# tomoyoshki/focal

Hardware: AMD Instinct MI355X
Metric: pretrain windows/sec (whole node), FOCAL SW_Transformer (higher is better)
Workload: dtype bf16

## Files before the change

### focal_amd/csrc/fft.hip

```cpp
#include <stdlib.h>
#include <type_traits>
#include "common.hpp"

struct AugParams {
  float scale, pc, ps;
  int flip, use_perm;
  int perm[FOCAL_AUG_MAX_INTERVALS];
  const focal_view_plan* plan;
  const float* x_alt;
};
static AugParams aug_identity() {
  AugParams a;
  memset(&a, 0, sizeof(a));
  a.scale = 1.f; a.pc = 1.f;
  return a;
}
struct AugLive {
  float scale, pc, ps;
  int flip, use_perm;
  const float* x;
};
__device__ __forceinline__ AugLive aug_resolve(const AugParams& a, const float* x, int* s_perm, int tid) {
  AugLive v{a.scale, a.pc, a.ps, a.flip, a.use_perm, x};
  if (a.plan != nullptr) {
    const focal_view_plan* pl = a.plan;
    v.scale = pl->aug.scale; v.pc = pl->aug.phase_cos; v.ps = pl->aug.phase_sin;
    v.flip = pl->aug.flip != 0; v.use_perm = pl->aug.use_perm != 0;
    if (focal_plan_warp(pl) != 0) v.x = a.x_alt;
    if (tid < FOCAL_AUG_MAX_INTERVALS) s_perm[tid] = pl->aug.perm[tid];
  } else if (tid < FOCAL_AUG_MAX_INTERVALS) {
    s_perm[tid] = a.perm[tid];
  }
  return v;
}
__device__ __forceinline__ int aug_src_row(const AugLive& a, const int* s_perm, int row, int I) {
  const int i = row % I, bc = row / I;
  int j = a.use_perm ? s_perm[i] : i;
  if (a.flip) j = I - 1 - j;
  return bc * I + j;
}


struct ExParams { const focal_view_extra* dev; int has; uint32_t salt; focal_view_extra host; };
template <bool EX> struct AugArg : AugParams {};
template <> struct AugArg<true> : AugParams { ExParams ex; };
struct ExLive {
  float std; uint32_t key;
  int any, use_chan, tlo, thi, flo, fhi;
};
__device__ __forceinline__ ExLive ex_resolve(const ExParams& p, int C, int n, int* s_chan, int tid) {
  float sd = 0.f;
  uint32_t key = 0u;
  int uc = 0, tlo = 0, tn = 0, flo = 0, fn = 0, ch = tid;
  if (p.dev != nullptr) {
    const focal_view_extra* e = p.dev;
    sd = e->jitter_std; key = e->jitter_key; uc = e->use_chan; tlo = e->tmask_lo; tn = e->tmask_n; flo = e->fmask_lo; fn = e->fmask_n;
    if (tid < FOCAL_VIEW_MAX_CHANNELS) ch = e->chan[tid];
  } else if (p.has) {
    sd = p.host.jitter_std; key = p.host.jitter_key; uc = p.host.use_chan; tlo = p.host.tmask_lo; tn = p.host.tmask_n;
    flo = p.host.fmask_lo; fn = p.host.fmask_n;
    if (tid < FOCAL_VIEW_MAX_CHANNELS) ch = p.host.chan[tid];
  }
  if (tid < FOCAL_VIEW_MAX_CHANNELS) s_chan[tid] = min(max(ch, 0), C - 1);
  ExLive v;
  v.std = sd > 0.f ? sd : 0.f;
  v.key = focal_mix32(key ^ focal_mix32(p.salt * 0x9E3779B9U + 0x85EBCA6BU));
  v.use_chan = uc != 0 && C <= FOCAL_VIEW_MAX_CHANNELS;
  v.tlo = min(max(tlo, 0), n); v.thi = v.tlo + min(max(tn, 0), n - v.tlo);
  v.flo = min(max(flo, 0), n); v.fhi = v.flo + min(max(fn, 0), n - v.flo);
  v.any = v.std > 0.f || v.use_chan || v.thi > v.tlo || v.fhi > v.flo;
  return v;
}
__device__ __forceinline__ int ex_src_row(const AugLive& a, const ExLive& ex, const int* s_perm, const int* s_chan, int row, int I, int C) {
  const int i = row % I;
  int bc = row / I;
  int j = a.use_perm ? s_perm[i] : i;
  if (a.flip) j = I - 1 - j;
  if (ex.use_chan) {
    const int c = bc % C;
    bc += s_chan[c] - c;
  }
  return bc * I + j;
}
__device__ __forceinline__ void ex_noise_pair(uint32_t k, uint32_t p, float& z0, float& z1) {
  const float u1 = 1.0f - (focal_mix32(k + (2u * p) * 0x85EBCA6BU) >> 8) * (1.0f / 16777216.0f);
  const float u2 = (focal_mix32(k + (2u * p + 1u) * 0x85EBCA6BU) >> 8) * (1.0f / 16777216.0f);
  const float r = sqrtf(-2.0f * __logf(u1)), a = 6.283185307179586f * u2;
  z0 = r * __cosf(a);
  z1 = r * __sinf(a);
}
__device__ __forceinline__ float ex_noise(uint32_t k, uint32_t e) {
  float z0, z1;
  ex_noise_pair(k, e >> 1, z0, z1);
  return (e & 1u) ? z1 : z0;
}

typedef float f4 __attribute__((ext_vector_type(4)));
__device__ __forceinline__ f4 mfma4(float a, float b, f4 c) { return __builtin_amdgcn_mfma_f32_16x16x4f32(a, b, c, 0, 0, 0); }

#define FFT_MULTI_MAX 8
struct FftSmallProblem { const float* x; const float* tw; float* out; int rows, I, n, rpb; AugParams aug; };
struct FftSmallExtraProblem : FftSmallProblem { int C; ExParams ex; };
template <bool EX> struct FftSmallTable { int nprob; int wg_end[FFT_MULTI_MAX]; std::conditional_t<EX, FftSmallExtraProblem, FftSmallProblem> p[FFT_MULTI_MAX]; };
static_assert(sizeof(FftSmallTable<true>) <= 4096, "the problem table travels in the kernel arguments");

template <bool EX>
__global__ __launch_bounds__(256) void fft_realpack_kernel(const float* __restrict__ x_arg, const float* __restrict__ tw,
                                                           float* __restrict__ out, focal_fft_desc d, int rows, AugArg<EX> aug_arg) {
  extern __shared__ __attribute__((aligned(16))) float smem[];
  __shared__ int s_perm[FOCAL_AUG_MAX_INTERVALS];
  const AugLive aug = aug_resolve(aug_arg, x_arg, s_perm, threadIdx.x);
  const float* x = aug.x;
  const int n = d.n, n1 = d.n1, n2 = d.n2;
  const int* s_chan = nullptr;
  ExLive ex{};
  if constexpr (EX) {
    __shared__ int chan_tab[FOCAL_VIEW_MAX_CHANNELS];
    ex = ex_resolve(aug_arg.ex, d.C, n, chan_tab, threadIdx.x);
    s_chan = chan_tab;
  }
  float* xs = smem;
  float* yr = smem + n;
  float* yi = yr + n;
  float* twc = yi + n;
  float* tws = twc + n;
  const int tid = threadIdx.x;
  for (int i = tid; i < n; i += 256) {
    twc[i] = tw[2 * i];
    tws[i] = tw[2 * i + 1];
  }
  for (int row = blockIdx.x; row < rows; row += gridDim.x) {
    __syncthreads();
    if (EX && ex.any) {
      const float* xr = x + (long)ex_src_row(aug, ex, s_perm, s_chan, row, d.I, d.C) * n;
      const uint32_t e0 = (uint32_t)row * (uint32_t)n;
      for (int i = tid; i < n; i += 256) {
        float v = aug.scale * xr[aug.flip ? n - 1 - i : i];
        if (ex.std > 0.f) v += ex.std * ex_noise(ex.key, e0 + (uint32_t)i);
        xs[i] = (i >= ex.tlo && i < ex.thi) ? 0.f : v;
      }
    } else {
      const float* xr = x + (long)aug_src_row(aug, s_perm, row, d.I) * n;
      for (int i = tid; i < n; i += 256) xs[i] = aug.scale * xr[aug.flip ? n - 1 - i : i];
    }
    __syncthreads();
    for (int o = tid; o < n; o += 256) {
      const int m2 = o / n1, k1 = o % n1;
      float re = 0.f, im = 0.f;
      int ph = 0;
      for (int m1 = 0; m1 < n1; ++m1) {
        const float v = xs[n2 * m1 + m2];
        re += v * twc[ph * n2];
        im += v * tws[ph * n2];
        ph += k1;
        if (ph >= n1) ph -= n1;
      }
      const int t = (m2 * k1) % n;
      const float c = twc[t], s = tws[t];
      yr[o] = re * c - im * s;
      yi[o] = re * s + im * c;
    }
    __syncthreads();
    const int ci = row % d.I, bc = row / d.I;
    float* ore = out + ((long)(2 * bc) * d.I + ci) * n;
    float* oim = out + ((long)(2 * bc + 1) * d.I + ci) * n;
    for (int o = tid; o < n; o += 256) {
      const int k = o, k1 = k % n1, k2 = k / n1;
      float re = 0.f, im = 0.f;
      int ph = 0;
      for (int m2 = 0; m2 < n2; ++m2) {
        const float a = yr[m2 * n1 + k1], b = yi[m2 * n1 + k1];
        const float c = twc[ph * n1], s = tws[ph * n1];
        re += a * c - b * s;
        im += a * s + b * c;
        ph += k2;
        if (ph >= n2) ph -= n2;
      }
      float orr = re * aug.pc - im * aug.ps, oii = re * aug.ps + im * aug.pc;
      if (EX && k >= ex.flo && k < ex.fhi) orr = oii = 0.f;
      ore[k] = orr;
      oim[k] = oii;
    }
  }
}
template <int N1, int N2, bool EX>
__global__ __launch_bounds__(256) void fft_realpack_mfma_kernel(const float* __restrict__ x_arg, const float* __restrict__ tw,
                                                                float* __restrict__ out, focal_fft_desc d, int rows, AugArg<EX> aug_arg) {
  constexpr int P = 48;
  extern __shared__ __attribute__((aligned(16))) float smem[];
  __shared__ int s_perm[FOCAL_AUG_MAX_INTERVALS];
  const AugLive aug = aug_resolve(aug_arg, x_arg, s_perm, threadIdx.x);
  const float* x = aug.x;
  constexpr int n = N1 * N2, n1 = N1, n2 = N2;
  const int* s_chan = nullptr;
  ExLive ex{};
  if constexpr (EX) {
    __shared__ int chan_tab[FOCAL_VIEW_MAX_CHANNELS];
    ex = ex_resolve(aug_arg.ex, d.C, n, chan_tab, threadIdx.x);
    s_chan = chan_tab;
  }
  float* twc = smem;
  float* tws = twc + n;
  float* w1c = tws + n;
  float* w1s = w1c + n1 * P;
  constexpr bool same = n1 == n2;
  float* w2c = same ? w1c : w1s + n1 * P;
  float* w2s = same ? w1s : w2c + n2 * P;
  float* yr = (same ? w1s : w2s) + n2 * P;
  float* yi = yr + 2 * n2 * P;
  float* xs = yi + 2 * n2 * P;
  const int tid = threadIdx.x, lane = tid & 63, wave = tid >> 6;
  const int lj = lane & 15, lg = lane >> 4;
  for (int i = tid; i < n; i += 256) { twc[i] = tw[2 * i]; tws[i] = tw[2 * i + 1]; }
  for (int i = tid; i < n1 * P; i += 256) {
    const int m = i / P, k = i % P;
    const int t = ((m * k) % n1) * n2;
    w1c[i] = k < n1 ? tw[2 * t] : 0.f;
    w1s[i] = k < n1 ? tw[2 * t + 1] : 0.f;
  }
  for (int i = tid; i < (same ? 0 : n2 * P); i += 256) {
    const int m = i / P, k = i % P;
    const int t = ((m * k) % n2) * n1;
    w2c[i] = k < n2 ? tw[2 * t] : 0.f;
    w2s[i] = k < n2 ? tw[2 * t + 1] : 0.f;
  }
  constexpr int mt1 = 2 * n2 / 16, mt2 = 2 * n1 / 16;
  constexpr int XV = (2 * n / 4 + 255) / 256;
  float4 xn[XV];
  auto fetch = [&](int pair) {
#pragma unroll
    for (int i = 0; i < XV; ++i) {
      const int e = tid + 256 * i;
      float4 v = make_float4(0.f, 0.f, 0.f, 0.f);
      if (e < 2 * n / 4 && pair < rows / 2) {
        const int rl = e / (n / 4), q = e - rl * (n / 4);
        const int srow = (EX && ex.any) ? ex_src_row(aug, ex, s_perm, s_chan, pair * 2 + rl, d.I, d.C) : aug_src_row(aug, s_perm, pair * 2 + rl, d.I);
        const float4* src = reinterpret_cast<const float4*>(x + (long)srow * n);
        if (aug.flip) {
          const float4 t = src[n / 4 - 1 - q];
          v = make_float4(t.w, t.z, t.y, t.x);
        } else {
          v = src[q];
        }
        v.x *= aug.scale; v.y *= aug.scale; v.z *= aug.scale; v.w *= aug.scale;
        if (EX && ex.any) {
          if (ex.std > 0.f) {
            const uint32_t p0 = ((uint32_t)(pair * 2 + rl) * (uint32_t)n + 4u * (uint32_t)q) >> 1;
            float z0, z1, z2, z3;
            ex_noise_pair(ex.key, p0, z0, z1);
            ex_noise_pair(ex.key, p0 + 1u, z2, z3);
            v.x += ex.std * z0; v.y += ex.std * z1; v.z += ex.std * z2; v.w += ex.std * z3;
          }
          const int i0 = 4 * q;
          if (i0 >= ex.tlo && i0 < ex.thi) v.x = 0.f;
          if (i0 + 1 >= ex.tlo && i0 + 1 < ex.thi) v.y = 0.f;
          if (i0 + 2 >= ex.tlo && i0 + 2 < ex.thi) v.z = 0.f;
          if (i0 + 3 >= ex.tlo && i0 + 3 < ex.thi) v.w = 0.f;
        }
      }
      xn[i] = v;
    }
  };
  auto stash = [&]() {
#pragma unroll
    for (int i = 0; i < XV; ++i) {
      const int e = tid + 256 * i;
      if (e < 2 * n / 4) reinterpret_cast<float4*>(xs)[e] = xn[i];
    }
  };
  __syncthreads();
  fetch(blockIdx.x);
  stash();
  for (int pair = blockIdx.x; pair < rows / 2; pair += gridDim.x) {
    __syncthreads();
    const float* x0 = xs;
    constexpr int np1 = (n1 + 15) / 16, np2 = (n2 + 15) / 16;
    for (int u = wave; u < mt1 * np1; u += 4) {
      const int mt = u / np1, p = u - mt * np1;
      const int f = 16 * mt + lj, row = f / n2, m2 = f - row * n2;
      const float* xa = x0 + row * n + m2;
      float a[12];
#pragma unroll
      for (int ks = 0; ks < 12; ++ks) {
        const int m1 = 4 * ks + lg;
        a[ks] = m1 < n1 ? xa[n2 * m1] : 0.f;
      }
      {
        f4 re = {0.f, 0.f, 0.f, 0.f}, im = re, re2 = re, im2 = re;
#pragma unroll
        for (int ks = 0; ks < 12; ks += 2) {
          if (4 * ks >= n1) break;
          const int bi = (4 * ks + lg) * P + 16 * p + lj;
          re = mfma4(a[ks], w1c[bi], re);
          im = mfma4(a[ks], w1s[bi], im);
          if (4 * (ks + 1) < n1) {
            re2 = mfma4(a[ks + 1], w1c[bi + 4 * P], re2);
            im2 = mfma4(a[ks + 1], w1s[bi + 4 * P], im2);
          }
        }
        re += re2;
        im += im2;
        const int k1 = 16 * p + lj;
        if (k1 < n1) {
#pragma unroll
          for (int r = 0; r < 4; ++r) {
            const int fo = 16 * mt + 4 * lg + r, ro = fo / n2, mo = fo - ro * n2;
            const int t = (mo * k1) % n;
            const float c = twc[t], sn = tws[t];
            yr[(ro * n2 + mo) * P + k1] = re[r] * c - im[r] * sn;
            yi[(ro * n2 + mo) * P + k1] = re[r] * sn + im[r] * c;
          }
        }
      }
    }
    __syncthreads();
    fetch(pair + gridDim.x);
    for (int u = wave; u < mt2 * np2; u += 4) {
      const int mt = u / np2, p = u - mt * np2;
      const int f = 16 * mt + lj, row = f / n1, k1 = f - row * n1;
      const float* ya = yr + row * n2 * P + k1;
      const float* yb = yi + row * n2 * P + k1;
      const int fo = 16 * mt + 4 * lg, ro = fo / n1, ko = fo - ro * n1;
      const int grow = pair * 2 + ro;
      const int ci = grow % d.I, bc = grow / d.I;
      float* ore = out + ((long)(2 * bc) * d.I + ci) * n + ko;
      float* oim = out + ((long)(2 * bc + 1) * d.I + ci) * n + ko;
      {
        f4 re = {0.f, 0.f, 0.f, 0.f}, im = re, re2 = re, im2 = re;
#pragma unroll
        for (int ks = 0; ks < 12; ++ks) {
          if (4 * ks >= n2) break;
          const int m2 = 4 * ks + lg;
          const float ar = ya[m2 * P], ai = yb[m2 * P];
          const int bi = m2 * P + 16 * p + lj;
          const float c = w2c[bi], sn = w2s[bi];
          re = mfma4(ar, c, re);
          im = mfma4(ar, sn, im);
          re2 = mfma4(ai, -sn, re2);
          im2 = mfma4(ai, c, im2);
        }
        re += re2;
        im += im2;
        const int k2 = 16 * p + lj;
        if (k2 < n2) {
          f4 orr = re * aug.pc - im * aug.ps, oii = re * aug.ps + im * aug.pc;
          if (EX && ex.fhi > ex.flo) {
#pragma unroll
            for (int r = 0; r < 4; ++r) {
              const int k = ko + r + n1 * k2;
              if (k >= ex.flo && k < ex.fhi) { orr[r] = 0.f; oii[r] = 0.f; }
            }
          }
          *reinterpret_cast<float4*>(ore + n1 * k2) = make_float4(orr[0], orr[1], orr[2], orr[3]);
          *reinterpret_cast<float4*>(oim + n1 * k2) = make_float4(oii[0], oii[1], oii[2], oii[3]);
        }
      }
    }
    stash();
  }
}
template <bool EX>
__global__ __launch_bounds__(256) void fft_small_multi_kernel(const FftSmallTable<EX> t) {
  __shared__ float xs[256], twc[64], tws[64];
  const int b = blockIdx.x, tid = threadIdx.x;
  int pi = 0;
#pragma unroll
  for (int q = 0; q < FFT_MULTI_MAX - 1; ++q) pi += (q < t.nprob - 1 && b >= t.wg_end[q]) ? 1 : 0;
  const auto& P = t.p[pi];
  __shared__ int s_perm[FOCAL_AUG_MAX_INTERVALS];
  const AugLive aug = aug_resolve(P.aug, P.x, s_perm, tid);
  int Cc = 1;
  const int* s_chan = nullptr;
  ExLive ex{};
  if constexpr (EX) {
    __shared__ int chan_tab[FOCAL_VIEW_MAX_CHANNELS];
    Cc = P.C;
    ex = ex_resolve(P.ex, Cc, P.n, chan_tab, threadIdx.x);
    s_chan = chan_tab;
  }
  const int start = pi > 0 ? t.wg_end[pi - 1] : 0, nb = t.wg_end[pi] - start;
  const int n = P.n, rpb = P.rpb;
  if (tid < n) { twc[tid] = P.tw[2 * tid]; tws[tid] = P.tw[2 * tid + 1]; }
  const int r = tid / n, k = tid - r * n;
  const bool active = r < rpb;
  for (int row0 = (b - start) * rpb; row0 < P.rows; row0 += nb * rpb) {
    const int row = row0 + r;
    const bool ok = active && row < P.rows;
    __syncthreads();
    if (EX && ex.any) {
      if (ok) {
        float v = aug.scale * aug.x[(long)ex_src_row(aug, ex, s_perm, s_chan, row, P.I, Cc) * n + (aug.flip ? n - 1 - k : k)];
        if (ex.std > 0.f) v += ex.std * ex_noise(ex.key, (uint32_t)row * (uint32_t)n + (uint32_t)k);
        xs[tid] = (k >= ex.tlo && k < ex.thi) ? 0.f : v;
      }
    } else if (ok) {
      xs[tid] = aug.scale * aug.x[(long)aug_src_row(aug, s_perm, row, P.I) * n + (aug.flip ? n - 1 - k : k)];
    }
    __syncthreads();
    if (!ok) continue;
    const float* xr = xs + r * n;
    float re = 0.f, im = 0.f;
    int ph = 0;
    for (int m = 0; m < n; ++m) {
      const float v = xr[m];
      re += v * twc[ph];
      im += v * tws[ph];
      ph += k;
      if (ph >= n) ph -= n;
    }
    const int ci = row % P.I, bc = row / P.I;
    float orr = re * aug.pc - im * aug.ps, oii = re * aug.ps + im * aug.pc;
    if (EX && k >= ex.flo && k < ex.fhi) orr = oii = 0.f;
    P.out[((long)(2 * bc) * P.I + ci) * n + k] = orr;
    P.out[((long)(2 * bc + 1) * P.I + ci) * n + k] = oii;
  }
}

template <bool EX>
static int fft_launch_t(const focal_fft_desc* d, const AugArg<EX>& aug, const float* x, const float* twiddle, float* out, void* stream) {
  FOCAL_CHECK_ARG(d && x && twiddle && out, "fft_realpack: null argument");
  FOCAL_CHECK_ARG(d->n1 >= 1 && d->n2 >= 1 && d->n1 * d->n2 == d->n, "fft_realpack: n1*n2 != n");
  const size_t sm = (size_t)5 * d->n * sizeof(float);
  FOCAL_CHECK_ARG(sm <= 64 * 1024, "fft_realpack: n=%d too long for the LDS-resident DFT", d->n);
  const int rows = d->B * d->C * d->I;
  const bool mfma_shape = (d->n1 == d->n2) && (d->n1 == 8 || d->n1 == 16 || d->n1 == 24 || d->n1 == 32 || d->n1 == 40 || d->n1 == 48);
  if (mfma_shape && rows % 2 == 0) {
    const size_t smm = (size_t)(2 * d->n + 2 * 48 * d->n1 + (d->n1 == d->n2 ? 0 : 2 * 48 * d->n2) + 4 * 48 * d->n2 + 2 * d->n) * sizeof(float);
    static size_t lds_granted = 48 * 1024;
    if (smm > lds_granted) {
      hipError_t e = hipSuccess;
#define FFT_ATTR(N_) if (e == hipSuccess) e = hipFuncSetAttribute(reinterpret_cast<const void*>(fft_realpack_mfma_kernel<N_, N_, EX>), hipFuncAttributeMaxDynamicSharedMemorySize, (int)smm)
      FFT_ATTR(8); FFT_ATTR(16); FFT_ATTR(24); FFT_ATTR(32); FFT_ATTR(40); FFT_ATTR(48);
#undef FFT_ATTR
      if (e != hipSuccess) {
        focal_set_error("fft_realpack: cannot reserve %zu bytes of LDS: %s", smm, hipGetErrorString(e));
        return FOCAL_EHIP;
      }
      lds_granted = smm;
    }
    const int maxb = 1024;
    int blocks = rows / 2 < maxb ? rows / 2 : maxb;
#define FFT_GO(N_) case N_: FOCAL_LAUNCH((fft_realpack_mfma_kernel<N_, N_, EX>), dim3(blocks), dim3(256), smm, (hipStream_t)stream, x, twiddle, out, *d, rows, aug); break
    switch (d->n1) { FFT_GO(8); FFT_GO(16); FFT_GO(24); FFT_GO(32); FFT_GO(40); default: FFT_GO(48); }
#undef FFT_GO
    FOCAL_LAUNCH_CHECK();
    return FOCAL_OK;
  }
  int blocks = rows < 4096 ? rows : 4096;
  FOCAL_LAUNCH(fft_realpack_kernel<EX>, dim3(blocks), dim3(256), sm, (hipStream_t)stream, x, twiddle, out, *d, rows, aug);
  FOCAL_LAUNCH_CHECK();
  return FOCAL_OK;
}

static int aug_params(const focal_fft_desc* d, const focal_aug_desc* a, AugParams* p) {
  *p = aug_identity();
  if (a == nullptr) return FOCAL_OK;
  p->scale = a->scale;
  p->flip = a->flip != 0;
  p->use_perm = a->use_perm != 0;
  p->pc = a->phase_cos;
  p->ps = a->phase_sin;
  if (p->use_perm) {
    FOCAL_CHECK_ARG(d->I <= FOCAL_AUG_MAX_INTERVALS, "augment_fft: %d intervals exceed the permutation table (%d)", d->I, FOCAL_AUG_MAX_INTERVALS);
    for (int i = 0; i < d->I; ++i) {
      FOCAL_CHECK_ARG(a->perm[i] >= 0 && a->perm[i] < d->I, "augment_fft: permutation entry %d out of range", a->perm[i]);
      p->perm[i] = a->perm[i];
    }
  }
  return FOCAL_OK;
}

static int ex_params(const focal_fft_problem& q, int i, ExParams* e) {
  memset(e, 0, sizeof(*e));
  e->salt = q.noise_salt;
  if (q.extra_dev != nullptr) {
    e->dev = q.extra_dev;
    return FOCAL_OK;
  }
  if (!q.has_extra) return FOCAL_OK;
  const focal_view_extra& x = q.extra;
  const int C = q.d.C, n = q.d.n;
  FOCAL_CHECK_ARG(x.jitter_std >= 0.f, "fft_realpack_multi: negative jitter std in problem %d", i);
  FOCAL_CHECK_ARG(x.tmask_lo >= 0 && x.tmask_n >= 0 && x.tmask_lo <= n && x.tmask_n <= n - x.tmask_lo, "fft_realpack_multi: time mask [%d, +%d) of problem %d leaves [0, %d]", x.tmask_lo, x.tmask_n, i, n);
  FOCAL_CHECK_ARG(x.fmask_lo >= 0 && x.fmask_n >= 0 && x.fmask_lo <= n && x.fmask_n <= n - x.fmask_lo, "fft_realpack_multi: freq mask [%d, +%d) of problem %d leaves [0, %d]", x.fmask_lo, x.fmask_n, i, n);
  if (x.use_chan) {
    FOCAL_CHECK_ARG(C <= FOCAL_VIEW_MAX_CHANNELS, "fft_realpack_multi: %d channels exceed the channel table (%d)", C, FOCAL_VIEW_MAX_CHANNELS);
    unsigned seen = 0;
    for (int c = 0; c < C; ++c) {
      FOCAL_CHECK_ARG(x.chan[c] >= 0 && x.chan[c] < C && !(seen >> x.chan[c] & 1u), "fft_realpack_multi: chan of problem %d is not a permutation of range(%d)", i, C);
      seen |= 1u << x.chan[c];
    }
  }
  e->has = 1;
  e->host = x;
  return FOCAL_OK;
}

template <bool EX>
static int fft_multi(int n, const focal_fft_problem* probs, void* stream) {
  FftSmallTable<EX> t;
  memset(&t, 0, sizeof(t));
  auto flush = [&]() -> int {
    if (t.nprob == 0) return FOCAL_OK;
    FOCAL_LAUNCH(fft_small_multi_kernel<EX>, dim3(t.wg_end[t.nprob - 1]), dim3(256), 0, (hipStream_t)stream, t);
    FOCAL_LAUNCH_CHECK();
    memset(&t, 0, sizeof(t));
    return FOCAL_OK;
  };
  for (int i = 0; i < n; ++i) {
    const focal_fft_problem& q = probs[i];
    FOCAL_CHECK_ARG(q.x && q.twiddle && q.out, "fft_realpack_multi: null tensor in problem %d", i);
    FOCAL_CHECK_ARG(q.d.B > 0 && q.d.C > 0 && q.d.I > 0 && q.d.n > 0, "fft_realpack: bad shape");
    AugArg<EX> ap;
    if (int rc = aug_params(&q.d, q.has_aug ? &q.aug : nullptr, &ap)) return rc;
    if constexpr (EX)
      if (int rc = ex_params(q, i, &ap.ex)) return rc;
    if (q.plan != nullptr) {
      FOCAL_CHECK_ARG(q.x_warped != nullptr && q.d.I <= FOCAL_AUG_MAX_INTERVALS, "fft_realpack_multi: a device plan needs x_warped and at most %d intervals", FOCAL_AUG_MAX_INTERVALS);
      ap.plan = q.plan;
      ap.x_alt = q.x_warped;
    }
    if (q.d.n <= 64 && q.d.n2 == 1 && q.d.n1 == q.d.n) {
      auto& P = t.p[t.nprob];
      if constexpr (EX) { P.C = q.d.C; P.ex = ap.ex; }
      P.x = q.x; P.tw = q.twiddle; P.out = q.out;
      P.rows = q.d.B * q.d.C * q.d.I; P.I = q.d.I; P.n = q.d.n; P.rpb = 256 / q.d.n;
      P.aug = ap;
      int blocks = ceil_div(P.rows, P.rpb);
      if (blocks > 1024) blocks = 1024;
      t.wg_end[t.nprob] = (t.nprob ? t.wg_end[t.nprob - 1] : 0) + blocks;
      if (++t.nprob == FFT_MULTI_MAX)
        if (int rc = flush()) return rc;
    } else if (int rc = fft_launch_t<EX>(&q.d, ap, q.x, q.twiddle, q.out, stream)) {
      return rc;
    }
  }
  return flush();
}

extern "C" int focal_fft_realpack_multi(int n, const focal_fft_problem* probs, void* stream) {
  FOCAL_CHECK_ARG(n >= 1 && probs, "fft_realpack_multi: no problems");
  bool ex = false;
  for (int i = 0; i < n; ++i) ex = ex || probs[i].has_extra || probs[i].extra_dev != nullptr;
  return ex ? fft_multi<true>(n, probs, stream) : fft_multi<false>(n, probs, stream);
}

extern "C" int focal_fft_realpack_fwd(const focal_fft_desc* d, const float* x, const float* twiddle, float* out, void* stream) {
  return fft_launch_t<false>(d, AugArg<false>{aug_identity()}, x, twiddle, out, stream);
}

extern "C" int focal_augment_fft_fwd(const focal_fft_desc* d, const focal_aug_desc* a, const float* x, const float* twiddle, float* out,
                                     void* stream) {
  FOCAL_CHECK_ARG(d && a, "augment_fft: null descriptor");
  AugArg<false> p;
  if (int rc = aug_params(d, a, &p)) return rc;
  return fft_launch_t<false>(d, p, x, twiddle, out, stream);
}
```

Measured before the change: 51920.

## Keep DFT twiddle matrices in registers and drop LDS twiddle tables

The square-factorisation MFMA FFT kernel no longer stages twiddle and DFT-matrix tables in LDS. Each lane precomputes its DFT coefficients once into registers and reuses them for both passes, and the inter-stage twiddles are read directly from global memory. Work is reassigned per column-tile with wave-uniform scheduling, and sched barriers and explicit non-contracted FMAs preserve rounding. This cuts LDS footprint and LDS traffic, at the cost of more registers and global twiddle loads.

New measurement: 52020 (median of 6 runs). Within noise of the previous version (+0.2%).

```diff
diff --git a/focal_amd/csrc/fft.hip b/focal_amd/csrc/fft.hip
--- a/focal_amd/csrc/fft.hip
+++ b/focal_amd/csrc/fft.hip
@@ -183,9 +183,20 @@
     }
   }
 }
+__device__ __forceinline__ float fft_mul_sub(float a, float b, float c, float d) {
+#pragma clang fp contract(off)
+  const float t = c * d;
+  return fmaf(a, b, -t);
+}
+__device__ __forceinline__ float fft_mul_add(float a, float b, float c, float d) {
+#pragma clang fp contract(off)
+  const float t = a * b;
+  return fmaf(c, d, t);
+}
 template <int N1, int N2, bool EX>
 __global__ __launch_bounds__(256) void fft_realpack_mfma_kernel(const float* __restrict__ x_arg, const float* __restrict__ tw,
                                                                 float* __restrict__ out, focal_fft_desc d, int rows, AugArg<EX> aug_arg) {
+  static_assert(N1 == N2 && N1 % 8 == 0 && N1 <= 48, "square factorisations, side a multiple of 8 up to 48");
   constexpr int P = 48;
   extern __shared__ __attribute__((aligned(16))) float smem[];
   __shared__ int s_perm[FOCAL_AUG_MAX_INTERVALS];
@@ -199,32 +210,29 @@
     ex = ex_resolve(aug_arg.ex, d.C, n, chan_tab, threadIdx.x);
     s_chan = chan_tab;
   }
-  float* twc = smem;
-  float* tws = twc + n;
-  float* w1c = tws + n;
-  float* w1s = w1c + n1 * P;
-  constexpr bool same = n1 == n2;
-  float* w2c = same ? w1c : w1s + n1 * P;
-  float* w2s = same ? w1s : w2c + n2 * P;
-  float* yr = (same ? w1s : w2s) + n2 * P;
+  float* yr = smem;
   float* yi = yr + 2 * n2 * P;
   float* xs = yi + 2 * n2 * P;
-  const int tid = threadIdx.x, lane = tid & 63, wave = tid >> 6;
+  const int tid = threadIdx.x, lane = tid & 63, wave = __builtin_amdgcn_readfirstlane(tid >> 6);
   const int lj = lane & 15, lg = lane >> 4;
-  for (int i = tid; i < n; i += 256) { twc[i] = tw[2 * i]; tws[i] = tw[2 * i + 1]; }
-  for (int i = tid; i < n1 * P; i += 256) {
-    const int m = i / P, k = i % P;
-    const int t = ((m * k) % n1) * n2;
-    w1c[i] = k < n1 ? tw[2 * t] : 0.f;
-    w1s[i] = k < n1 ? tw[2 * t + 1] : 0.f;
-  }
-  for (int i = tid; i < (same ? 0 : n2 * P); i += 256) {
-    const int m = i / P, k = i % P;
-    const int t = ((m * k) % n2) * n1;
-    w2c[i] = k < n2 ? tw[2 * t] : 0.f;
-    w2s[i] = k < n2 ? tw[2 * t + 1] : 0.f;
-  }
+  constexpr int KS = n1 / 4;
+  constexpr int np1 = (n1 + 15) / 16, np2 = np1;
   constexpr int mt1 = 2 * n2 / 16, mt2 = 2 * n1 / 16;
+  float wc[np1][KS], ws[np1][KS];
+#pragma unroll
+  for (int p = 0; p < np1; ++p) {
+    const int k = 16 * p + lj;
+    const int step = (4 * k) % n1;
+    int ph = (lg * k) % n1;
+#pragma unroll
+    for (int ks = 0; ks < KS; ++ks) {
+      const int t = 2 * ph * n2;
+      wc[p][ks] = k < n1 ? tw[t] : 0.f;
+      ws[p][ks] = k < n1 ? tw[t + 1] : 0.f;
+      ph += step;
+      if (ph >= n1) ph -= n1;
+    }
+  }
   constexpr int XV = (2 * n / 4 + 255) / 256;
   float4 xn[XV];
   auto fetch = [&](int pair) {
@@ -273,77 +281,92 @@
   stash();
   for (int pair = blockIdx.x; pair < rows / 2; pair += gridDim.x) {
     __syncthreads();
-    const float* x0 = xs;
-    constexpr int np1 = (n1 + 15) / 16, np2 = (n2 + 15) / 16;
-    for (int u = wave; u < mt1 * np1; u += 4) {
-      const int mt = u / np1, p = u - mt * np1;
-      const int f = 16 * mt + lj, row = f / n2, m2 = f - row * n2;
-      const float* xa = x0 + row * n + m2;
-      float a[12];
-#pragma unroll
-      for (int ks = 0; ks < 12; ++ks) {
-        const int m1 = 4 * ks + lg;
-        a[ks] = m1 < n1 ? xa[n2 * m1] : 0.f;
-      }
-      {
+    int tz = 0;
+    asm volatile("" : "+s"(tz));
+#pragma unroll
+    for (int p = 0; p < np1; ++p) {
+#pragma unroll 1
+      for (int mt = 0; mt < mt1; ++mt) {
+        if (((mt * np1 + p) & 3) != wave) continue;
+        const int f = 16 * mt + lj, row = f / n2, m2 = f - row * n2;
+        const float* xa = xs + row * n + m2;
+        float a[KS];
+#pragma unroll
+        for (int ks = 0; ks < KS; ++ks) a[ks] = xa[n2 * (4 * ks + lg)];
+        const int k1 = 16 * p + lj;
+        float tc[4], ts[4];
+#pragma unroll
+        for (int r = 0; r < 4; ++r) {
+          const int fo = 16 * mt + 4 * lg + r, mo = fo - (fo / n2) * n2;
+          const int t = (k1 < n1 ? 2 * mo * k1 : 0) + tz;
+          tc[r] = tw[t];
+          ts[r] = tw[t + 1];
+        }
+        __builtin_amdgcn_sched_barrier(0);
         f4 re = {0.f, 0.f, 0.f, 0.f}, im = re, re2 = re, im2 = re;
 #pragma unroll
-        for (int ks = 0; ks < 12; ks += 2) {
-          if (4 * ks >= n1) break;
-          const int bi = (4 * ks + lg) * P + 16 * p + lj;
-          re = mfma4(a[ks], w1c[bi], re);
-          im = mfma4(a[ks], w1s[bi], im);
-          if (4 * (ks + 1) < n1) {
-            re2 = mfma4(a[ks + 1], w1c[bi + 4 * P], re2);
-            im2 = mfma4(a[ks + 1], w1s[bi + 4 * P], im2);
-          }
+        for (int ks = 0; ks < KS; ks += 2) {
+          re = mfma4(a[ks], wc[p][ks], re);
+          im = mfma4(a[ks], ws[p][ks], im);
+          re2 = mfma4(a[ks + 1], wc[p][ks + 1], re2);
+          im2 = mfma4(a[ks + 1], ws[p][ks + 1], im2);
         }
         re += re2;
         im += im2;
-        const int k1 = 16 * p + lj;
         if (k1 < n1) {
 #pragma unroll
           for (int r = 0; r < 4; ++r) {
-            const int fo = 16 * mt + 4 * lg + r, ro = fo / n2, mo = fo - ro * n2;
-            const int t = (mo * k1) % n;
-            const float c = twc[t], sn = tws[t];
-            yr[(ro * n2 + mo) * P + k1] = re[r] * c - im[r] * sn;
-            yi[(ro * n2 + mo) * P + k1] = re[r] * sn + im[r] * c;
+            const int fo = 16 * mt + 4 * lg + r;
+            yr[fo * P + k1] = fft_mul_sub(re[r], tc[r], im[r], ts[r]);
+            yi[fo * P + k1] = fft_mul_add(re[r], ts[r], im[r], tc[r]);
           }
         }
       }
     }
     __syncthreads();
     fetch(pair + gridDim.x);
-    for (int u = wave; u < mt2 * np2; u += 4) {
-      const int mt = u / np2, p = u - mt * np2;
-      const int f = 16 * mt + lj, row = f / n1, k1 = f - row * n1;
-      const float* ya = yr + row * n2 * P + k1;
-      const float* yb = yi + row * n2 * P + k1;
-      const int fo = 16 * mt + 4 * lg, ro = fo / n1, ko = fo - ro * n1;
+    float* orow[2];
+#pragma unroll
+    for (int ro = 0; ro < 2; ++ro) {
       const int grow = pair * 2 + ro;
       const int ci = grow % d.I, bc = grow / d.I;
-      float* ore = out + ((long)(2 * bc) * d.I + ci) * n + ko;
-      float* oim = out + ((long)(2 * bc + 1) * d.I + ci) * n + ko;
-      {
+      orow[ro] = out + ((long)(2 * bc) * d.I + ci) * n;
+    }
+    const long im_off = (long)d.I * n;
+#pragma unroll
+    for (int p = 0; p < np2; ++p) {
+#pragma unroll 1
+      for (int mt = 0; mt < mt2; ++mt) {
+        if (((mt * np2 + p) & 3) != wave) continue;
+        const int f = 16 * mt + lj, row = f / n1, k1 = f - row * n1;
+        const float* ya = yr + (row * n2 + lg) * P + k1;
+        const float* yb = yi + (row * n2 + lg) * P + k1;
+        float ar[KS], ai[KS];
+#pragma unroll
+        for (int ks = 0; ks < KS; ++ks) {
+          ar[ks] = ya[4 * ks * P];
+          ai[ks] = yb[4 * ks * P];
+        }
+        __builtin_amdgcn_sched_barrier(0);
         f4 re = {0.f, 0.f, 0.f, 0.f}, im = re, re2 = re, im2 = re;
 #pragma unroll
-        for (int ks = 0; ks < 12; ++ks) {
-          if (4 * ks >= n2) break;
-          const int m2 = 4 * ks + lg;
-          const float ar = ya[m2 * P], ai = yb[m2 * P];
-          const int bi = m2 * P + 16 * p + lj;
-          const float c = w2c[bi], sn = w2s[bi];
-          re = mfma4(ar, c, re);
-          im = mfma4(ar, sn, im);
-          re2 = mfma4(ai, -sn, re2);
-          im2 = mfma4(ai, c, im2);
+        for (int ks = 0; ks < KS; ++ks) {
+          re = mfma4(ar[ks], wc[p][ks], re);
+          im = mfma4(ar[ks], ws[p][ks], im);
+          re2 = mfma4(-ai[ks], ws[p][ks], re2);
+          im2 = mfma4(ai[ks], wc[p][ks], im2);
         }
         re += re2;
         im += im2;
         const int k2 = 16 * p + lj;
         if (k2 < n2) {
-          f4 orr = re * aug.pc - im * aug.ps, oii = re * aug.ps + im * aug.pc;
+          const int fo = 16 * mt + 4 * lg, ro = fo / n1, ko = fo - ro * n1;
+          float orr[4], oii[4];
+#pragma unroll
+          for (int r = 0; r < 4; ++r) {
+            orr[r] = fft_mul_sub(re[r], aug.pc, im[r], aug.ps);
+            oii[r] = fft_mul_add(re[r], aug.ps, im[r], aug.pc);
+          }
           if (EX && ex.fhi > ex.flo) {
 #pragma unroll
             for (int r = 0; r < 4; ++r) {
@@ -351,8 +374,9 @@
               if (k >= ex.flo && k < ex.fhi) { orr[r] = 0.f; oii[r] = 0.f; }
             }
           }
-          *reinterpret_cast<float4*>(ore + n1 * k2) = make_float4(orr[0], orr[1], orr[2], orr[3]);
-          *reinterpret_cast<float4*>(oim + n1 * k2) = make_float4(oii[0], oii[1], oii[2], oii[3]);
+          float* ore = (ro ? orow[1] : orow[0]) + ko + n1 * k2;
+          *reinterpret_cast<float4*>(ore) = make_float4(orr[0], orr[1], orr[2], orr[3]);
+          *reinterpret_cast<float4*>(ore + im_off) = make_float4(oii[0], oii[1], oii[2], oii[3]);
         }
       }
     }
@@ -425,7 +449,7 @@
   const int rows = d->B * d->C * d->I;
   const bool mfma_shape = (d->n1 == d->n2) && (d->n1 == 8 || d->n1 == 16 || d->n1 == 24 || d->n1 == 32 || d->n1 == 40 || d->n1 == 48);
   if (mfma_shape && rows % 2 == 0) {
-    const size_t smm = (size_t)(2 * d->n + 2 * 48 * d->n1 + (d->n1 == d->n2 ? 0 : 2 * 48 * d->n2) + 4 * 48 * d->n2 + 2 * d->n) * sizeof(float);
+    const size_t smm = (size_t)(4 * 48 * d->n2 + 2 * d->n) * sizeof(float);
     static size_t lds_granted = 48 * 1024;
     if (smm > lds_granted) {
       hipError_t e = hipSuccess;
```
